# matteocarnelos/microflow-rs

Measured on AMD Instinct MI355X. Metric: inferences/sec (int8) for person_detect.tflite, higher is better.
Workload: dtype i8; 1 GPU; person_detect.tflite batch=65536 per GPU, predict_inner int8->int8, inputs resident in HBM; per_gpu_batch=65536, global_batch=65536, parallelism=batch shard x1, no data-path collective

## Files before the change

microflow_rs_amd/csrc/fused.hip:

```cpp
#include <algorithm>
#include <cmath>
#include <cstdio>
#include <cstring>
#include <memory>

#include "ops_impl.hpp"
#include "wimage.hpp"

namespace mf {

struct FusedImpl {
    enum Kind { DWPW, TAIL, FCSM, STAGE, DWFC, PAIRTAIL, QUAD, CHAIN, FCCHAIN, POOLFC } kind;
    OpImpl *a, *b, *c;
    k::DwPwArgs dwpw;
    k::TailArgs tail;
    std::string name;
    k::StageArgs stage{};
    int stage_pairs = 0;
    std::vector<std::unique_ptr<DevBuf>> stage_w;
    k::DwFcArgs dwfc{};
    k::PairTailArgs pairtail{};
    k::PairFrontArgs pairfront{};
    bool has_front = false;
    k::QuadArgs quad{};
// ... 464 lines not shown
    std::unique_ptr<FusedImpl> f(new FusedImpl{FusedImpl::PAIRTAIL, dw, pairtail->b, pairtail->c, {}, {}, "pair_front_tail<6,6,128,2,256|3,3,256,2>"});
    f->pairtail = t, f->has_front = true, f->epi_mode = magic;
    k::PairFrontArgs &a = f->pairfront;
    a.dw_wmm = df.wmm, a.dwA = df.A, a.dwS = df.S, a.dwK = magic ? kc_with_magic(*f, dw->h_Kc) : df.Kc;
    a.dw_lo = df.lo_f, a.dw_hi = df.hi_f, a.izp4 = df.izp4;
    a.pw_w = plain_pw_image(*f, pw);
    a.pwA = pw->conv.A, a.pwS = pw->conv.S, a.pwK = magic ? kc_with_magic(*f, pw->h_Kc) : pw->conv.Kc;
    a.pw_lo = pw->conv.lo_f, a.pw_hi = pw->conv.hi_f;
    return f.release();
}

static FusedImpl *quad_group(FusedImpl *p1, FusedImpl *p2, const k::DwPwArgs &a, const k::DwPwArgs &b, const char *name, bool mm) {
    const OpSpec &d1 = p1->a->s, &q1 = p1->b->s, &d2 = p2->a->s, &q2 = p2->b->s;
    FusedImpl *f = new FusedImpl{FusedImpl::QUAD, p1->a, p2->b, nullptr, {}, {}, name};
    f->quad.a = a, f->quad.b = b, f->quad_mm = mm;
    f->epi_mode = std::min(pair_mode(a), pair_mode(b));
    f->quad_ops[0] = p1->a, f->quad_ops[1] = p1->b, f->quad_ops[2] = p2->a, f->quad_ops[3] = p2->b;
    const int shp[10] = {d1.H, d1.W, d1.C, d1.sh, q1.N, d2.H, d2.W, d2.C, d2.sh, q2.N};
    for (int i = 0; i < 10; ++i) f->quad_shape[i] = shp[i];
    return f;
}
FusedImpl *fused_quad_create(FusedImpl *p1, FusedImpl *p2) {
    const bool off = switches().no_quad;
    if (off || !p1 || !p2 || p1->kind != FusedImpl::DWPW || p2->kind != FusedImpl::DWPW) return nullptr;
    const OpSpec &d1 = p1->a->s, &q1 = p1->b->s, &d2 = p2->a->s, &q2 = p2->b->s;
    if (p1->a->device != p2->a->device || d1.u8 != d2.u8) return nullptr;
    if (d2.H != q1.H || d2.W != q1.W || d2.C != q1.N) return nullptr;
    if (k::quad_mm_shape(d1.H, d1.W, d1.C, d1.sh, q1.N, d2.H, d2.W, d2.C, d2.sh, q2.N)) {
        if (switches().no_quad_mm) return nullptr;
        k::DwPwArgs a = p1->dwpw, b = p2->dwpw;
        if (pair_mode(a) != 3 || pair_mode(b) != 3) a = pair_args(p1->a, p1->b, 0), b = pair_args(p2->a, p2->b, 0);
        if (!a.dw.wmm || !a.pw.wprep || !b.dw.wmm || !b.pw.wprep) return nullptr;
        if (!a.dw.magic || !a.pw.magic || !b.dw.magic || !b.pw.magic) return nullptr;
        return quad_group(p1, p2, a, b, "quad_mm<12,12,64,1,64|12,12,64,2,128>", true);
    }
    const char *nm = k::quad_name(d1.H, d1.W, d1.C, d1.sh, q1.N, d2.H, d2.W, d2.C, d2.sh, q2.N);
    if (!nm) return nullptr;
    const bool fma = p1->a->fma_strict() && p1->b->fma_strict() && p2->a->fma_strict() && p2->b->fma_strict();
    const k::DwPwArgs a = pair_args(p1->a, p1->b, fma ? 1 : 0), b = pair_args(p2->a, p2->b, fma ? 1 : 0);
    if (!a.dw.wmm || !a.pw.wrr || !b.dw.wmm || !b.pw.wrr) return nullptr;
    if (!a.dw.magic || !a.pw.magic || !b.dw.magic || !b.pw.magic) return nullptr;
    return quad_group(p1, p2, a, b, nm, false);
}

FusedImpl *fused_quad_stem_create(OpImpl *stem, FusedImpl *quad) {
    const bool off = switches().no_penta;
    if (off || !stem || !quad || quad->kind != FusedImpl::QUAD || quad->quad.stem || stem->fast != OpImpl::DW_STEM) return nullptr;
    const OpSpec &t = stem->s, &d1 = quad->a->s;
    if (stem->device != quad->a->device || t.u8 != d1.u8 || stem->force_generic) return nullptr;
    if (t.OH != d1.H || t.OW != d1.W || t.N != d1.C || t.sh != 2 || t.sw != 2 || t.C != 1) return nullptr;
    const int *q = quad->quad_shape;
    const char *nm = k::quad_stem_name(t.H, t.W, q[0], q[1], q[2], q[3], q[4], q[5], q[6], q[7], q[8], q[9]);
    if (!nm || !stem->stem.magic) return nullptr;
    std::unique_ptr<FusedImpl> f(new FusedImpl{FusedImpl::QUAD, stem, quad->b, nullptr, {}, {}, nm});
    f->quad = quad->quad;
    for (int i = 0; i < 10; ++i) f->quad_shape[i] = q[i];
    OpImpl *const *qo = quad->quad_ops;
    const bool fma = stem->fma_strict() && qo[0]->fma_strict() && qo[1]->fma_strict() && qo[2]->fma_strict() && qo[3]->fma_strict();
    f->quad.a = pair_args(qo[0], qo[1], fma ? 1 : 0), f->quad.b = pair_args(qo[2], qo[3], fma ? 1 : 0);
    k::DwStemArgs sa = stem->stem;
    if (fma) sa.use_fma();
    std::vector<uint32_t> tab(152);
    for (int l = 0; l < 64; ++l) tab[(size_t)2 * l] = sa.wmm[l][0], tab[(size_t)2 * l + 1] = sa.wmm[l][1];
    for (int c = 0; c < 8; ++c) {
        memcpy(&tab[(size_t)128 + c], &sa.A[c], 4);
        memcpy(&tab[(size_t)136 + c], &sa.S[c], 4);
        memcpy(&tab[(size_t)144 + c], &sa.Kc[c], 4);
// ... 358 lines not shown
```

microflow_rs_amd/csrc/k_quad_mm.hip:

```cpp
#include "k_common.hpp"

#ifndef MF_QMM_UB
#define MF_QMM_UB 2
#endif
#ifndef MF_QMM_KO
#define MF_QMM_KO 0
#endif
namespace mf {
namespace k {

namespace {
struct Q64 {
    static constexpr int G = 2, NTHR = 512, NWAVE = 8, NQ = 4, LP = 64, ROWB = 768;
    static constexpr int ROW_A = LP + ROWB + LP + 16, TILE_A = 14 * ROW_A, BUF_A = G * TILE_A;
    static constexpr int OPIX_A = 144, NPIX_A = G * OPIX_A, PLANE_A = NPIX_A * 16 + 16;
    static constexpr int ROW_B = LP + ROWB + LP, TILE_B = 14 * ROW_B, BUF_B = G * TILE_B, TS_B = 0x043;
    static constexpr int OPIX_B = 36, NPIX_B = G * OPIX_B, P16_B = 80, PLANE_B = P16_B * 16 + 16;
    static constexpr int OFF_TA = 0;
    static constexpr int OFF_MA = OFF_TA + BUF_A + 512;
    static constexpr int OFF_TB = OFF_MA + NQ * PLANE_A + 64;
    static constexpr int OFF_MB = OFF_TB + BUF_B + 512;
    static constexpr int OFF_C = OFF_MB + NQ * PLANE_B + 64;
    static constexpr int C_A_DW = 0, C_A_PW = 64 * 12, C_B_DW = 2 * 64 * 12, C_B_PW = 3 * 64 * 12, C_BYTES = 3 * 64 * 12 + 128 * 12;
    static constexpr int OFF_Q = OFF_C + C_BYTES;
    static constexpr int LDS = OFF_Q + 16;
};
static_assert(2 * Q64::LDS <= 160 * 1024, "two workgroups per CU");
static_assert(Q64::OFF_MA % 16 == 0 && Q64::OFF_TB % 16 == 0 && Q64::OFF_MB % 16 == 0, "16-byte aligned regions");
}

template <int MG, uint32_t XR4>
__global__ __launch_bounds__(512, 4) void quad_mm_12x12x64(const int8_t *__restrict__ in, int8_t *__restrict__ out, QuadArgs p, int batch) {
    using Z = Q64;
    constexpr int UB = MF_QMM_UB;
    epi_enter<MG>();
    extern __shared__ __attribute__((aligned(16))) uint8_t lds[];
// ... 181 lines not shown
                                                    : requant_pack4<MG, XR4>(acc[t][0], acc[t][1], acc[t][2], acc[t][3], k.a, k.s, p.b.dw.lo_f, p.b.dw.hi_f);
                if (liveB) *(uint32_t *)(lds + mbB + t * 2 * 6 * 16) = d;
            }
        }
        if (!(MF_QMM_KO & 1)) wg_sync();

        if (!(MF_QMM_KO & 4)) {
            constexpr int NC = 5;
            const Consts k = consts(Z::C_B_PW, 128, chB);
            v4i b[NC], acc[NC];
#pragma unroll
            for (int c = 0; c < NC; ++c) {
                const int pix = c * 16 + col, pc = pix < Z::NPIX_B ? pix : Z::NPIX_B - 1;
                b[c] = *(const v4i *)(lds + Z::OFF_MB + g * Z::PLANE_B + pc * 16);
            }
#pragma unroll
            for (int c = 0; c < NC; ++c) acc[c] = __builtin_amdgcn_mfma_i32_16x16x64_i8(AwB, b[c], v4i{k.k.x, k.k.y, k.k.z, k.k.w}, 0, 0, 0);
#pragma unroll
            for (int c = 0; c < NC; ++c) {
                const int pix = c * 16 + col;
                if constexpr (MG == 3) epi_patch_apply(acc[c], prPB, g);
                const uint32_t d = (MF_QMM_KO & 16) ? (uint32_t)(acc[c][0] ^ acc[c][1] ^ acc[c][2] ^ acc[c][3])
                                                    : requant_pack4<MG, XR4>(acc[c][0], acc[c][1], acc[c][2], acc[c][3], k.a, k.s, p.b.pw.lo_f, p.b.pw.hi_f);
                if (pix < Z::NPIX_B) *(uint32_t *)(lds + out_addr(pix, blk * 4 + g) + 4 * tt) = d;
            }
        }
        prev = step, prev_gv = gvalid;
    }
    wg_sync();
    if (prev >= 0) copy_out(prev, prev_gv);
    dq.finish(tid);
}

template <int MG, uint32_t XR4> static void launch_quad_mm_t(const int8_t *in, int8_t *out, const QuadArgs &a, int batch, hipStream_t s) {
    static LaunchState st;
    const int per_cu = prepared(st, quad_mm_12x12x64<MG, XR4>, Q64::NTHR, Q64::LDS);
    const int nsteps = (batch + Q64::G - 1) / Q64::G;
    const int grid = nsteps < 256 * per_cu ? nsteps : 256 * per_cu;
    QuadArgs b = a;
    b.a.dw.qcfg = dq_config(nsteps, grid, dq_est_us((double)batch * (9216 + 4608), (double)batch * (9216 * 2 + 2304 + 4608)));
    b.a.dw.queue = dq_slot(b.a.dw.queue, b.a.dw.qlaunch);
    hipLaunchKernelGGL((quad_mm_12x12x64<MG, XR4>), dim3(grid), dim3(Q64::NTHR), Q64::LDS, s, in, out, b, batch);
}
bool quad_mm_shape(int H, int W, int C, int S, int N, int H2, int W2, int C2, int S2, int N2) {
    return H == 12 && W == 12 && C == 64 && S == 1 && N == 64 && H2 == 12 && W2 == 12 && C2 == 64 && S2 == 2 && N2 == 128;
}
void launch_quad_mm(const int8_t *in, int8_t *out, const QuadArgs &a, int batch, hipStream_t s) {
    const int mg = std::min(std::min(a.a.dw.magic, a.a.pw.magic), std::min(a.b.dw.magic, a.b.pw.magic));
    const bool u8 = a.a.dw.xr != 0;
    if (mg == 3) launch_quad_mm_t<3, 0u>(in, out, a, batch, s);
    else if (u8) {
        if (mg == 2) launch_quad_mm_t<2, 0x80808080u>(in, out, a, batch, s);
        else launch_quad_mm_t<1, 0x80808080u>(in, out, a, batch, s);
    } else {
        if (mg == 2) launch_quad_mm_t<2, 0u>(in, out, a, batch, s);
        else launch_quad_mm_t<1, 0u>(in, out, a, batch, s);
    }
}

}
}
```

microflow_rs_amd/csrc/kernels.hpp:

```cpp
#pragma once
#include <hip/hip_runtime.h>
#include <stddef.h>
#include <stdint.h>

#include <vector>

namespace mf {
namespace k {

struct ConvArgs {
    int H, W, C;
    int N;
    int KH, KW, sh, sw, OH, OW;
    int pad_same;
    int izp;
    float lo_f, hi_f;
    const int8_t *w;
    const int *wzp;
    const float *A;
    const float *S;
    const int *Kc;
    int xr;
};
struct PoolArgs {
// ... 248 lines not shown
    const ChainPair *pairs;
    int npairs, G;
    int lds_bytes, mid_off, q_off;
    int dbuf, dbuf_stride;
    int stage_after;
    int nfill;
    int fill_off[CHAIN_MAX], fill_bytes[CHAIN_MAX];
    uint32_t fill_izp4[CHAIN_MAX];
    int *queue;
    unsigned long *qlaunch;
    int qcfg;
    int KSC;
    int max_cg;
    int resident;
    int nwave;
    double est_us_per_image;
    int magic, xr;
    double hbm_bytes, requant_bytes;
};
bool chain_plan(const ChainGeom *g, int n, ChainPair *pairs, ChainArgs &a, int lds_budget, int force_G = 0, int force_dbuf = -1);
double chain_unfused_us_per_image(const ChainGeom *g, int n);
void chain_rtab(const ChainPair &c, std::vector<int> &out);
void launch_chain(const int8_t *in, int8_t *out, const ChainArgs &a, int batch, hipStream_t s);

struct QuadArgs {
    DwPwArgs a, b;
    const uint32_t *stem;
    uint32_t stem_izp4;
    float stem_lo, stem_hi;
    int stem_magic;
    float in_scale, in_zp_f, in_sat_lo, in_sat_hi, in_rcp;
    uint32_t in_xr4;
    int in_fast, f32_ok;
};
const char *quad_name(int H, int W, int C, int S, int N, int H2, int W2, int C2, int S2, int N2);
const char *quad_stem_name(int SH, int SW, int H, int W, int C, int S, int N, int H2, int W2, int C2, int S2, int N2);
bool launch_quad(int H, int W, int C, int S, int N, int H2, int W2, int C2, int S2, int N2, const int8_t *in, int8_t *out, const QuadArgs &a,
                 int batch, hipStream_t s);
bool quad_mm_shape(int H, int W, int C, int S, int N, int H2, int W2, int C2, int S2, int N2);
void launch_quad_mm(const int8_t *in, int8_t *out, const QuadArgs &a, int batch, hipStream_t s);
bool launch_quad_f32(int H, int W, int C, int S, int N, int H2, int W2, int C2, int S2, int N2, const float *in, int8_t *out, const QuadArgs &a,
                     int batch, hipStream_t s);

struct TailArgs {
    int H, W, C, N;
    int ntaps;
    int tap_off[64];
    float inv_len;
    float pool_c0, pool_c1;
    int pool_lo, pool_hi;
    const int8_t *w;
    const int *wzp;
    const float *A;
    const float *S;
    const int *Kc;
    float lo_f, hi_f;
    const float *exp_table;
    float sm_oscale, sm_ozp_f;
    int pool_bias;
    float pool_sat_lo, pool_sat_hi, sm_sat_lo, sm_sat_hi;
    int xr;
};

struct DwFcGeom {
    static constexpr int H = 49, W = 40, KH = 10, KW = 8, S = 2, OH = 25, OW = 20;
    static constexpr int IMGS = 16;
// ... 291 lines not shown
```

microflow_rs_amd/csrc/mf_switches.hpp:

```cpp
#pragma once
#include <string>
#include <vector>

namespace mf {

struct ChainPlanSeg {
    int len;
    int G;
    int dbuf;
};
bool chain_plan_parse(const char *text, std::vector<ChainPlanSeg> &out, std::string &err);

struct Switches {
    bool dev = false;
    bool no_rt = false;
    bool no_stem_rt = false;
    bool no_chain = false;
    bool chain_no_sp = false;
    bool no_stage = false;
    bool no_fc_rt = false;
    bool no_fc_sparse = false;
    bool no_fc_chain = false;
    bool no_pool_fc = false;
    bool no_conv_gemm = false;
    bool no_dw_gemm = false;
    bool no_dwfc = false;
    bool no_pairtail = false;
    bool no_pair_front = false;
    bool no_quad_mm = false;
    bool no_quad = false;
    bool no_penta = false;
    bool no_f32_group = false;
    int quads = 7;
    bool no_magic = false;
    bool no_sat_pack = false;
    bool no_table = false;
    bool chain_all = false;
    bool chain_force = false;
    bool chain_no_res = false;
    bool conv_mm_256 = false;
    bool no_fma_epi = false;
    bool no_fast_quant_div = false;
    bool dwpw_mm_only = false;
    bool stem_valu = false;
    bool dw_c1_lds = false;
    int dw_alt = -1;
    int dwmm_alt = -1;
    int dwrr_alt = -1;
    int fc_tile = 0;
    bool fc_rowsum_fold = false;
    bool fc_rowsum_prepass = false;
    long long pw_grid = 0;
    int pw_rt_ncap = 64;
    int dw_rt_threads = 0;
    int chain_autotune = -1;
    bool chain_tune_g = true;
    double chain_opcost = 1.0;
    bool chain_dq_auto = false;
    bool chain_plan_set = false;
    std::vector<ChainPlanSeg> chain_plan;
    std::string chain_plan_error;
    bool dq_tune = false;
// ... 15 lines not shown
```

microflow_rs_amd/csrc/ops.hip:

```cpp
#include <algorithm>
#include <array>
#include <cmath>
#include <cstdio>
#include <cstdlib>
#include <cstring>
#include <map>
#include <memory>
#include <mutex>

#include "ops_impl.hpp"
#include "wimage.hpp"

namespace mf {

int dev_count() {
    int n = 0;
    if (hipGetDeviceCount(&n) != hipSuccess) {
        (void)hipGetLastError();
        return 0;
    }
    return n;
}

void dev_require(int device) {
// ... 277 lines not shown
    k::DwC1Args &f = op.dwc1;
    f.H = s.H, f.W = s.W, f.N = s.N, f.KH = s.KH, f.KW = s.KW, f.sh = s.sh, f.sw = s.sw;
    f.OH = s.OH, f.OW = s.OW, f.pad_same = s.pad == MF_PAD_SAME, f.izp = s.izp;
    f.A = op.conv.A, f.S = op.conv.S, f.Kc = op.conv.Kc;
    epi_fields(f, op, c);
    f.KG = (s.KW + 3) / 4;
    f.TWP = ((((s.OW - 1) * s.sw + 3) & ~3) + 4 * (f.KG + 1) + 3) & ~3;
    if (k::dw_c1_supported(f)) {
        op.h_wpack = wimage::build_dw_c1_pack(s.weights, s.KH, s.KW, s.N, f.KG);
        op.d_wprep.upload(op.h_wpack.data(), op.h_wpack.size() * 4);
        f.wpack = op.d_wprep.as<uint32_t>();
        op.fast = OpImpl::DW_C1;
        op.fast_name = "dw_c1_lds";
    }
    return true;
}

bool route_pw_mfma(OpImpl &op, const ConvCtx &c) {
    const OpSpec &s = c.s;
    if (!(!switches().no_table && !c.dw && c.zero_wzp && s.KH == 1 && s.KW == 1 && s.sh == 1 && s.sw == 1 &&
          s.OH == s.H && s.OW == s.W && k::pw_name(s.C, s.N) &&
          (s.C != 8 || ((s.H * s.W) % 2 == 0))))
        return false;
    op.fast = OpImpl::PW_MFMA;
    op.fast_name = k::pw_name(s.C, s.N);
    const std::vector<int8_t> prep = wimage::build_pw_weights(s.weights, s.C, s.N);
    op.d_wprep.upload(prep.data(), prep.size());
    k::PwArgs &f = op.pw;
    f.wprep = op.d_wprep.p, f.A = op.conv.A, f.S = op.conv.S, f.Kc = op.conv.Kc;
    epi_fields(f, op, c);
    f.wrr = nullptr;
    if ((s.C == 8 || s.C == 16 || s.C == 32) && (s.C == 8 ? 2 * s.N : s.N) % 16 == 0) {
        const std::vector<int8_t> rr = wimage::build_pw_rr_weights(s.weights, s.C, s.N);
        op.d_wrr.upload(rr.data(), rr.size());
        f.wrr = op.d_wrr.p;
    }
    return true;
}

bool rt_candidate(const OpImpl &op, const ConvCtx &c) {
    const bool no_rt = switches().no_rt;
    return op.fast == OpImpl::NONE && !no_rt && c.finite;
}

bool route_dw_rt(OpImpl &op, const ConvCtx &c) {
    const OpSpec &s = c.s;
    if (!(rt_candidate(op, c) && c.dw && c.same3x3 && s.C == s.N && k::dw_rt_plan(op.dwrt, s.H, s.W, s.C, s.sh, s.OH, s.OW))) return false;
    op.fast = OpImpl::DW_RT;
    op.rt_wz = c.wz;
    op.fast_name = std::string("dw3x3_rt<") + std::to_string(s.sh) + (op.rt_wz ? ",wzp>" : ">");
    k::DwFastArgs &f = op.dwrt.dw;
    f.w = op.conv.w, f.A = op.conv.A, f.S = op.conv.S, f.Kc = op.conv.Kc, f.wmm = nullptr;
    epi_fields_izp(f, op, c);
    step_queue(f, op);
    op.dwrt.wzp = op.conv.wzp;
    if (!op.rt_wz && (s.C % 16 == 0 || s.C == 8)) {
        const std::vector<int8_t> prep = wimage::build_dw_mm_weights(s.weights, s.C);
        op.d_wprep.upload(prep.data(), prep.size());
        f.wmm = op.d_wprep.p;
    }
    return true;
}

bool route_pw_rt(OpImpl &op, const ConvCtx &c) {
    const OpSpec &s = c.s;
    if (!(rt_candidate(op, c) && !c.dw && s.KH == 1 && s.KW == 1 && s.sh == 1 && s.sw == 1 && s.OH == s.H && s.OW == s.W)) return false;
// ... 658 lines not shown
```

microflow_rs_amd/csrc/switches.cpp:

```cpp
#include "mf_switches.hpp"
#include <cstdlib>
#include <string>

namespace mf {

static bool env_set(const char *name) { return getenv(name) != nullptr; }
static bool env_is(const char *name, char first) { const char *e = getenv(name); return e && e[0] == first; }
static long long env_ll(const char *name, long long dflt) { const char *e = getenv(name); return e ? strtoll(e, nullptr, 0) : dflt; }

bool chain_plan_parse(const char *text, std::vector<ChainPlanSeg> &out, std::string &err) {
    out.clear(), err.clear();
    auto bad = [&](const std::string &why) {
        out.clear();
        err = why;
        return false;
    };
    if (!text || !*text) return bad("empty plan");
    const char *p = text;
    for (;;) {
        int v[3];
        for (int f = 0; f < 3; ++f) {
            const bool neg = *p == '-';
            const char *d = p + (neg ? 1 : 0);
            if (*d < '0' || *d > '9') return bad("entry " + std::to_string(out.size()) + ": expected len:G:dbuf");
// ... 15 lines not shown
        if (s.len == 0 && (s.G != 0 || s.dbuf != -1)) return bad(at + "an unfused pair (len 0) takes G 0 and dbuf -1");
        if (s.len >= 2 && s.dbuf != -1) return bad(at + "double buffering is a single pair's choice (len 1): a chain takes dbuf -1");
        out.push_back(s);
        if (!*p) return true;
        if (*p != ',') return bad(at + "expected ',' or the end");
        ++p;
    }
}

Switches switches_parse() {
    Switches s;
    s.verbose = env_set("MF_VERBOSE");
    s.chain_verbose = env_set("MF_CHAIN_VERBOSE");
    s.dq_verbose = env_set("MF_DQ_VERBOSE");
    s.debug_epi = env_set("MF_DEBUG_EPI");
    s.dev = env_is("MF_DEV", '1');
    if (!s.dev) return s;
    s.no_rt = env_set("MF_NO_RT");
    s.no_stem_rt = env_set("MF_NO_STEM_RT");
    s.no_chain = env_set("MF_NO_CHAIN");
    s.chain_no_sp = env_set("MF_CHAIN_NO_SP");
    s.no_stage = env_set("MF_NO_STAGE");
    s.no_dwfc = env_set("MF_NO_DWFC");
    s.no_fc_rt = env_set("MF_NO_FC_RT");
    s.no_fc_chain = env_set("MF_NO_FC_CHAIN");
    s.no_pool_fc = env_set("MF_NO_POOL_FC");
    s.no_conv_gemm = env_set("MF_NO_CONV_GEMM");
    s.no_dw_gemm = env_set("MF_NO_DW_GEMM");
    s.no_fc_sparse = env_set("MF_NO_FC_SPARSE");
    s.no_pairtail = env_set("MF_NO_PAIRTAIL");
    s.no_quad = env_set("MF_NO_QUAD");
    s.no_pair_front = env_set("MF_NO_PAIR_FRONT");
    s.no_quad_mm = env_set("MF_NO_QUAD_MM");
    s.no_penta = env_set("MF_NO_PENTA");
    s.no_f32_group = env_set("MF_NO_F32_GROUP");
    s.quads = (int)env_ll("MF_QUADS", 7);
    s.no_magic = env_set("MF_NO_MAGIC");
    s.no_sat_pack = env_set("MF_NO_SAT_PACK");
    s.no_table = env_set("MF_NO_TABLE");
    s.chain_all = env_set("MF_CHAIN_ALL");
    s.chain_force = env_set("MF_CHAIN_FORCE");
    s.chain_no_res = env_set("MF_CHAIN_NO_RES");
    s.conv_mm_256 = env_set("MF_CONV_MM_256");
    s.no_fma_epi = env_set("MF_NO_FMA_EPI");
    s.no_fast_quant_div = env_set("MF_NO_FAST_QUANT_DIV");
    s.dwpw_mm_only = env_is("MF_DWPW_IMPL", 'm');
    s.stem_valu = env_is("MF_STEM_IMPL", 'v');
    s.dw_c1_lds = env_is("MF_DW_C1", 'l');
    s.dw_alt = (int)env_ll("MF_DW_ALT", -1);
    s.dwmm_alt = (int)env_ll("MF_DWMM_ALT", -1);
    s.dwrr_alt = (int)env_ll("MF_DWRR_ALT", -1);
    s.fc_tile = (int)env_ll("MF_FC_TILE", 0);
    s.fc_rowsum_fold = env_set("MF_FC_ROWSUM_FOLD");
    s.fc_rowsum_prepass = env_set("MF_FC_ROWSUM_PREPASS");
    s.pw_grid = env_ll("MF_PW_GRID", 0);
    s.pw_rt_ncap = (int)env_ll("MF_PW_RT_NCAP", 64);
    s.dw_rt_threads = (int)env_ll("MF_DW_RT_THREADS", 0);
    s.chain_autotune = !env_set("MF_CHAIN_AUTOTUNE") ? -1 : (env_is("MF_CHAIN_AUTOTUNE", '0') ? 0 : 1);
    s.chain_tune_g = !env_is("MF_CHAIN_TUNE_G", '0');
    if (const char *e = getenv("MF_CHAIN_OPCOST")) s.chain_opcost = atof(e);
    s.chain_dq_auto = env_set("MF_CHAIN_DQ_AUTO");
    if (const char *e = getenv("MF_CHAIN_PLAN")) s.chain_plan_set = true, chain_plan_parse(e, s.chain_plan, s.chain_plan_error);
    s.dq_tune = env_set("MF_DQ_TUNE");
    s.dq_cfg_set = env_set("MF_DQ_CFG");
    s.dq_cfg = (int)env_ll("MF_DQ_CFG", 0);
    if (const char *l = getenv("MF_DQ_CFGS")) s.dq_cfgs = l;
// ... 11 lines not shown
```

microflow_rs_amd/csrc/wimage.cpp:

```cpp
#include "wimage.hpp"

#include <cstring>

namespace mf {
namespace wimage {

std::vector<int8_t> build_pw_weights(const int8_t *w , int K, int N) {
    const int NB = N < 64 ? N : 64, TB = NB / 16, NSPLIT = N / NB;
    const int KS = K < 64 ? 1 : K / 64, Q = K < 64 ? 64 / K : 1;
    std::vector<int8_t> out((size_t)NSPLIT * Q * TB * KS * 64 * 16, 0);
    for (int blk = 0; blk < NSPLIT; ++blk)
        for (int q = 0; q < Q; ++q)
            for (int tt = 0; tt < TB; ++tt)
                for (int ks = 0; ks < KS; ++ks)
                    for (int lane = 0; lane < 64; ++lane) {
                        const int r = lane & 15, g = lane >> 4;
                        const int gr = r >> 2, j = r & 3;
                        const int ch = blk * NB + gr * (NB / 4) + 4 * tt + j;
                        int8_t *dst = &out[(((((size_t)blk * Q + q) * TB + tt) * KS + ks) * 64 + lane) * 16];
                        for (int i = 0; i < 16; ++i) {
                            int k = -1;
                            if (K >= 64) k = ks * 64 + g * 16 + i;
                            else if (K == 32) k = ((g >> 1) == q) ? (g & 1) * 16 + i : -1;
                            else if (K == 16) k = (g == q) ? i : -1;
// ... 81 lines not shown
            for (int pp = 0; pp < P; ++pp) {
                const int tx = P * (g - 1) + pp - S * p + 1;
                if (g < 3 && tx >= 0 && tx <= 2) dst[pp * C + c] = w[(ty * 3 + tx) * C + c];
            }
        }
    return out;
}

std::vector<int8_t> build_pw_rr_weights(const int8_t *w , int K, int N) {
    const bool pair = K == 8;
    const int NT = (pair ? 2 * N : N) / 16;
    std::vector<int8_t> out((size_t)NT * 64 * 8, 0);
    for (int m = 0; m < NT; ++m)
        for (int lane = 0; lane < 64; ++lane) {
            const int r = lane & 15, g = lane >> 4;
            const int gr = r >> 2, i = r & 3;
            const int n = pair ? 8 * (gr & 1) + 4 * m + i : (N / 4) * gr + 4 * m + i;
            int8_t *dst = &out[((size_t)m * 64 + lane) * 8];
            for (int b = 0; b < 8; ++b) {
                int k = -1;
                if (pair) {
                    if (b < 4 && (g >> 1) == (gr >> 1)) k = 4 * (g & 1) + b;
                } else if (b < 4) {
                    k = 4 * g + b;
                } else if (K == 32) {
                    k = 16 + 4 * g + (b - 4);
                }
                dst[b] = k >= 0 && n < N ? w[(size_t)n * K + k] : (int8_t)0;
            }
        }
    return out;
}

std::vector<int8_t> build_pw_rt_weights(const int8_t *w , int K, int N, int group, bool ones) {
    const int Kg = K * group, Ng = N * group, KS = (Kg + 63) / 64, NT = (Ng + 15) / 16;
    std::vector<int8_t> out(((size_t)NT * KS + (ones ? KS : 0)) * 1024, 0);
    for (int nt = 0; nt < NT; ++nt)
        for (int ks = 0; ks < KS; ++ks)
            for (int lane = 0; lane < 64; ++lane) {
                const int row = 16 * nt + (lane & 15), g = lane >> 4;
                if (row >= Ng) continue;
                const int gi = row / N, n = row % N;
                int8_t *dst = &out[(((size_t)nt * KS + ks) * 64 + lane) * 16];
                for (int i = 0; i < 16; ++i) {
                    const int kk = ks * 64 + g * 16 + i;
                    if (kk < Kg && kk / K == gi) dst[i] = w[(size_t)n * K + kk % K];
                }
            }
    if (ones) fill_ones_tile(&out[(size_t)NT * KS * 1024], Kg, KS);
    return out;
}

std::vector<int8_t> build_pw_rt_reg_weights(const int8_t *w , int K, int N, int group, int TB, int NBLK) {
    const int Kg = K * group, Ng = N * group, KS = (Kg + 63) / 64;
    std::vector<int8_t> out((size_t)NBLK * TB * KS * 1024, 0);
    for (int blk = 0; blk < NBLK; ++blk)
        for (int t = 0; t < TB; ++t)
            for (int ks = 0; ks < KS; ++ks)
                for (int lane = 0; lane < 64; ++lane) {
                    const int r = lane & 15, g = lane >> 4;
                    const int row = 16 * TB * blk + 4 * TB * (r >> 2) + 4 * t + (r & 3);
                    if (row >= Ng) continue;
                    const int gi = row / N, n = row % N;
                    int8_t *dst = &out[((((size_t)blk * TB + t) * KS + ks) * 64 + lane) * 16];
                    for (int i = 0; i < 16; ++i) {
                        const int kk = ks * 64 + g * 16 + i;
// ... 67 lines not shown
```

microflow_rs_amd/csrc/wimage.hpp:

```cpp
#pragma once
#include <cstddef>
#include <cstdint>
#include <vector>

namespace mf {
namespace wimage {

std::vector<int8_t> build_pw_weights(const int8_t *w , int K, int N);
std::vector<int8_t> build_dw_mm_weights(const int8_t *w , int C);
std::vector<int8_t> build_dw_sp_weights(const std::vector<int8_t> &dense , int NQ);
std::vector<int8_t> build_dw_mm_rt_weights(const int8_t *w, int KH, int KW, int C, int KS ,
                                           int P = 1);
std::vector<int8_t> build_dw_mm_weights_sp(const int8_t *w , int C, int S);
std::vector<int8_t> build_pw_rr_weights(const int8_t *w , int K, int N);
std::vector<int8_t> build_pw_rt_weights(const int8_t *w , int K, int N, int group, bool ones);
std::vector<int8_t> build_pw_rt_reg_weights(const int8_t *w , int K, int N, int group, int TB, int NBLK);
std::vector<int8_t> build_pw_plain_weights(const int8_t *w, int K, int N);

void fill_ones_tile(int8_t *dst , int K, int KS);
void build_stem_rows(const int8_t *w , int N, uint32_t wrow[3][8]);
void build_stem_mm(const int8_t *w , int N, uint32_t *wmm , int pitch);
std::vector<uint32_t> build_conv_rows_pack(const int8_t *w, bool depthwise, int KH, int KW, int C, int N, int KG, int NP);
inline std::vector<uint32_t> build_dw_c1_pack(const int8_t *w , int KH, int KW, int N, int KG) { return build_conv_rows_pack(w, true, KH, KW, 1, N, KG, 8); }
std::vector<uint32_t> build_conv_rows_mask(int RWB , int KG);

}
}
```

Baseline: 29.78 million inferences/s.

## Add register-resident 64-channel quad_mm kernel that chains depthwise and pointwise outputs in registers

Adds a new variant of the 12x12x64 quad depthwise/pointwise kernel. It runs 256 threads with two workgroups per CU. The first-stage pointwise weights stay in registers, using a new rr64 weight layout for C=64, so the depthwise requantised output feeds the pointwise MFMA straight from registers instead of passing through LDS planes. The second-stage weights move into LDS, MFMA sections are wrapped in s_setprio, and the single epilogue patch is handled as a compile-time template parameter. The aims are to cut LDS traffic and intermediate staging and to raise occupancy, at the cost of higher register pressure and a more complex waitcnt/barrier schedule.

```diff
diff --git a/microflow_rs_amd/csrc/fused.hip b/microflow_rs_amd/csrc/fused.hip
--- a/microflow_rs_amd/csrc/fused.hip
+++ b/microflow_rs_amd/csrc/fused.hip
@@ -520,7 +520,17 @@
         if (pair_mode(a) != 3 || pair_mode(b) != 3) a = pair_args(p1->a, p1->b, 0), b = pair_args(p2->a, p2->b, 0);
         if (!a.dw.wmm || !a.pw.wprep || !b.dw.wmm || !b.pw.wprep) return nullptr;
         if (!a.dw.magic || !a.pw.magic || !b.dw.magic || !b.pw.magic) return nullptr;
-        return quad_group(p1, p2, a, b, "quad_mm<12,12,64,1,64|12,12,64,2,128>", true);
+        const k::EpiPatch &e1 = p1->b->fma_patch;
+        const bool rr = !switches().quad_mm_lds && pair_mode(a) == 3 && pair_mode(b) == 3 && a.pw.wrr && b.pw.wrr && q1.C == 64 && q2.C == 64 &&
+                        p1->a->fma_patch.n == 0 && p2->a->fma_patch.n == 0 && p2->b->fma_patch.n == 0 && e1.n <= 1;
+        FusedImpl *f = quad_group(p1, p2, a, b, rr ? "quad_mm<12,12,64,1,64|12,12,64,2,128>;rr" : "quad_mm<12,12,64,1,64|12,12,64,2,128>", true);
+        f->quad.rr64 = rr ? 1 : 0, f->quad.rr64_ptile = -1;
+        if (rr && e1.n == 1) {
+            const int ch = e1.ch[0];
+            f->quad.rr64_ptile = (ch & 15) >> 2, f->quad.rr64_preg = ch & 3, f->quad.rr64_pgrp = ch >> 4;
+            f->quad.rr64_pP = e1.P[0], f->quad.rr64_pR = e1.R[0];
+        }
+        return f;
     }
     const char *nm = k::quad_name(d1.H, d1.W, d1.C, d1.sh, q1.N, d2.H, d2.W, d2.C, d2.sh, q2.N);
     if (!nm) return nullptr;
diff --git a/microflow_rs_amd/csrc/k_quad_mm.hip b/microflow_rs_amd/csrc/k_quad_mm.hip
--- a/microflow_rs_amd/csrc/k_quad_mm.hip
+++ b/microflow_rs_amd/csrc/k_quad_mm.hip
@@ -1,7 +1,15 @@
 #include "k_common.hpp"
+
+#include <type_traits>
 
 #ifndef MF_QMM_UB
 #define MF_QMM_UB 2
+#endif
+#ifndef MF_R64_PRIO
+#define MF_R64_PRIO 1
+#endif
+#ifndef MF_R64_KO
+#define MF_R64_KO 0
 #endif
 #ifndef MF_QMM_KO
 #define MF_QMM_KO 0
@@ -249,6 +257,266 @@
     dq.finish(tid);
 }
 
+namespace {
+struct R64 {
+    static constexpr int G = 2, NTHR = 256, NWAVE = 4, LP = 64, ROWB = 768;
+    static constexpr int ROW_A = Q64::ROW_A, TILE_A = Q64::TILE_A, BUF_A = Q64::BUF_A;
+    static constexpr int ROW_B = Q64::ROW_B, TILE_B = Q64::TILE_B, BUF_B = Q64::BUF_B, TS_B = Q64::TS_B;
+    static constexpr int OFF_TA = 0, OFF_TB = BUF_A + 512, OFF_C = OFF_TB + BUF_B + 512;
+    static constexpr int C_A_DW = Q64::C_A_DW, C_A_PW = Q64::C_A_PW, C_B_DW = Q64::C_B_DW, C_B_PW = Q64::C_B_PW, C_BYTES = Q64::C_BYTES;
+    static constexpr int OFF_WD = OFF_C + C_BYTES, OFF_WP = OFF_WD + 12 * 1024;
+    static constexpr int OFF_Q = OFF_WP + 8 * 1024, LDS = OFF_Q + 16;
+};
+static_assert(2 * R64::LDS <= 160 * 1024 && R64::OFF_TB % 16 == 0 && R64::OFF_C % 16 == 0, "two workgroups per CU, 16-byte aligned regions");
+__device__ __forceinline__ void rr64_barrier_raw() {
+    mf_jitter();
+    asm volatile("s_waitcnt lgkmcnt(0)\n\ts_barrier" ::: "memory");
+    mf_jitter();
+}
+}
+
+template <int MG, uint32_t XR4, int PM>
+__global__ __launch_bounds__(256, 2) void quad_mm_12x12x64_rr(const int8_t *__restrict__ in, int8_t *__restrict__ out, QuadArgs p, int batch) {
+    using Z = R64;
+    static_assert(MG == 3 || PM < 0, "patched accumulators exist in the single-fma form only");
+    epi_enter<MG>();
+    extern __shared__ __attribute__((aligned(16))) uint8_t lds[];
+    const int tid = threadIdx.x, lane = tid & 63;
+    const int wave = __builtin_amdgcn_readfirstlane(tid >> 6);
+    DynSteps dq;
+    dq.init(lds + Z::OFF_Q, p.a.dw.queue, tid, p.a.dw.qcfg);
+    for (int i = tid; i < (Z::BUF_A + 512) / 16; i += Z::NTHR)
+        ((uint4 *)(lds + Z::OFF_TA))[i] = make_uint4(p.a.dw.izp4, p.a.dw.izp4, p.a.dw.izp4, p.a.dw.izp4);
+    for (int i = tid; i < (Z::BUF_B + 512) / 16; i += Z::NTHR)
+        ((uint4 *)(lds + Z::OFF_TB))[i] = make_uint4(p.b.dw.izp4, p.b.dw.izp4, p.b.dw.izp4, p.b.dw.izp4);
+    {
+        auto put = [&](int off, int n, const float *A, const float *S, const int *K) {
+            for (int i = tid; i < n; i += Z::NTHR) {
+                ((float *)(lds + Z::OFF_C + off))[i] = A[i], ((float *)(lds + Z::OFF_C + off))[n + i] = S[i];
+                ((int *)(lds + Z::OFF_C + off))[2 * n + i] = K[i] + (MG != 0 ? MF_MAGIC_I : 0);
+            }
+        };
+        put(Z::C_A_DW, 64, p.a.dw.A, p.a.dw.S, p.a.dw.Kc), put(Z::C_A_PW, 64, p.a.pw.A, p.a.pw.S, p.a.pw.Kc);
+        put(Z::C_B_DW, 64, p.b.dw.A, p.b.dw.S, p.b.dw.Kc), put(Z::C_B_PW, 128, p.b.pw.A, p.b.pw.S, p.b.pw.Kc);
+    }
+    struct Consts {
+        float4 a, s;
+        int4 k;
+    };
+    auto consts = [&](int off, int n, int ch) {
+        Consts c;
+        c.a = *(const float4 *)(lds + Z::OFF_C + off + ch * 4), c.s = *(const float4 *)(lds + Z::OFF_C + off + (n + ch) * 4);
+        c.k = *(const int4 *)(lds + Z::OFF_C + off + (2 * n + ch) * 4);
+        return c;
+    };
+    const int col = lane & 15, g = lane >> 4;
+    const int cyA = col & 3, cxA = col >> 2;
+    const int tbA = Z::OFF_TA + cyA * Z::ROW_A + Z::LP + (cxA + g - 1) * 64;
+    const int dbA = Z::OFF_TB + (cyA + 1) * Z::ROW_B + Z::LP + cxA * 64;
+    const int cxB = col & 7, cyB = col >> 3, xlB = cxB * 2 + g - 1;
+    int tbB[4];
+#pragma unroll
+    for (int q = 0; q < 4; ++q) tbB[q] = Z::OFF_TB + cyB * 2 * Z::ROW_B + Z::LP + xlB * 64 + 16 * (q ^ tile_swz<Z::TS_B>(xlB));
+    const int obB = (cyB * 6 + cxB) * 128 + 32 * g;
+    const bool liveB = cxB < 6;
+    const int rw = wave;
+    const bool xA = rw < 2, xB = rw >= 2;
+    int offA[5], dofA[5], swA[5], offB[2], oofB[2], hB[2];
+#pragma unroll
+    for (int t = 0; t < 5; ++t) {
+        const int iu = (t < 4 || xA) ? 4 * t + rw : rw, h = iu / 9, r = iu - 9 * h, uy = r / 3, ux = r - 3 * uy;
+        offA[t] = h * Z::TILE_A + uy * 4 * Z::ROW_A + ux * 256, dofA[t] = h * Z::TILE_B + uy * 4 * Z::ROW_B + ux * 256;
+        swA[t] = 16 * ux;
+    }
+#pragma unroll
+    for (int t = 0; t < 2; ++t) {
+        const int iu = t == 0 ? rw : (xB ? rw + 2 : rw), h = iu / 3, r = iu - 3 * h;
+        offB[t] = h * Z::TILE_B + r * 4 * Z::ROW_B, oofB[t] = (h * 36 + r * 12) * 128, hB[t] = h;
+    }
+    v4i AdA[4][3], AwA[4];
+#pragma unroll
+    for (int q = 0; q < 4; ++q)
+#pragma unroll
+        for (int ty = 0; ty < 3; ++ty) AdA[q][ty] = ((const v4i *)p.a.dw.wmm)[(q * 3 + ty) * 64 + lane];
+#pragma unroll
+    for (int m = 0; m < 4; ++m) AwA[m] = ((const v4i *)p.a.pw.wrr)[m * 64 + lane];
+    for (int i = tid; i < 12 * 64; i += Z::NTHR) ((v4i *)(lds + Z::OFF_WD))[i] = ((const v4i *)p.b.dw.wmm)[i];
+    for (int i = tid; i < 8 * 64; i += Z::NTHR) ((v4i *)(lds + Z::OFF_WP))[i] = ((const v4i *)p.b.pw.wrr)[i];
+    v4i pcmp = {0, 0, 0, 0};
+    if constexpr (PM >= 0) {
+        const int P = g == p.rr64_pgrp ? p.rr64_pP : 0;
+        pcmp = v4i{p.rr64_preg == 0 ? P : 0, p.rr64_preg == 1 ? P : 0, p.rr64_preg == 2 ? P : 0, p.rr64_preg == 3 ? P : 0};
+    }
+    const int prepl = p.rr64_pR;
+    wg_sync();
+
+    auto stage = [&](int st) {
+#pragma unroll
+        for (int k = 0; k < 6; ++k) {
+            const int r = k * Z::NWAVE + wave, gi = r / 12, y = r % 12;
+            if (st * Z::G + gi < batch && lane < 48)
+                dma16(in + ((size_t)(st * Z::G + gi) * 9216 + y * Z::ROWB + lane * 16), lds + Z::OFF_TA + gi * Z::TILE_A + (y + 1) * Z::ROW_A + Z::LP);
+        }
+    };
+    auto phase_a = [&](auto nu_c) {
+        constexpr int NU = decltype(nu_c)::value;
+        uint32_t d[NU][4], pk[NU][4];
+        v4i b[NU][3], bn[NU][3];
+        auto taps = [&](v4i (&t)[NU][3], int q) {
+#pragma unroll
+            for (int u = 0; u < NU; ++u)
+#pragma unroll
+                for (int ty = 0; ty < 3; ++ty) t[u][ty] = *(const v4i *)(lds + tbA + 16 * q + offA[u] + ty * Z::ROW_A);
+        };
+        taps(b, 0);
+        Consts k = consts(Z::C_A_DW, 64, 4 * g), kn = k;
+#pragma unroll
+        for (int q = 0; q < 4; ++q) {
+            v4i acc[NU];
+#pragma unroll
+            for (int u = 0; u < NU; ++u) acc[u] = v4i{k.k.x, k.k.y, k.k.z, k.k.w};
+#if MF_R64_PRIO
+            __builtin_amdgcn_s_setprio(MF_R64_PRIO);
+#endif
+#pragma unroll
+            for (int ty = 0; ty < 3; ++ty)
+#pragma unroll
+                for (int u = 0; u < NU; ++u) acc[u] = __builtin_amdgcn_mfma_i32_16x16x64_i8(AdA[q][ty], b[u][ty], acc[u], 0, 0, 0);
+#if MF_R64_PRIO
+            __builtin_amdgcn_s_setprio(0);
+#endif
+            if (q < 3) taps(bn, q + 1), kn = consts(Z::C_A_DW, 64, 16 * (q + 1) + 4 * g);
+            else kn = consts(Z::C_A_PW, 64, 16 * g);
+#pragma unroll
+            for (int u = 0; u < NU; ++u) d[u][q] = requant_pack4<MG, XR4>(acc[u][0], acc[u][1], acc[u][2], acc[u][3], k.a, k.s, p.a.dw.lo_f, p.a.dw.hi_f);
+#pragma unroll
+            for (int u = 0; u < NU; ++u)
+#pragma unroll
+                for (int ty = 0; ty < 3; ++ty) b[u][ty] = bn[u][ty];
+            k = kn;
+        }
+#pragma unroll
+        for (int m = 0; m < 4; ++m) {
+            v4i acc[NU];
+#pragma unroll
+            for (int u = 0; u < NU; ++u)
+                acc[u] = __builtin_amdgcn_mfma_i32_16x16x64_i8(AwA[m], v4i{(int)d[u][0], (int)d[u][1], (int)d[u][2], (int)d[u][3]}, v4i{k.k.x, k.k.y, k.k.z, k.k.w}, 0, 0, 0);
+            if (m < 3) kn = consts(Z::C_A_PW, 64, 16 * g + 4 * (m + 1));
+#pragma unroll
+            for (int u = 0; u < NU; ++u) {
+                if (PM == m && !MF_EPI_PATCH_KO) {
+#pragma unroll
+                    for (int j = 0; j < 4; ++j) acc[u][j] = acc[u][j] == pcmp[j] ? prepl : acc[u][j];
+                }
+                pk[u][m] = requant_pack4<MG, XR4>(acc[u][0], acc[u][1], acc[u][2], acc[u][3], k.a, k.s, p.a.pw.lo_f, p.a.pw.hi_f);
+            }
+            k = kn;
+        }
+#pragma unroll
+        for (int u = 0; u < NU; ++u) *(uint4 *)(lds + dbA + dofA[u] + ((16 * g) ^ swA[u])) = make_uint4(pk[u][0], pk[u][1], pk[u][2], pk[u][3]);
+    };
+    auto phase_b = [&](auto nu_c, int8_t *ob, int gvalid) {
+        constexpr int NU = decltype(nu_c)::value;
+        uint32_t d[NU][4], pk[NU][8];
+        v4i b[NU][3], bn[NU][3], Ad[3], Adn[3];
+        auto taps = [&](v4i (&t)[NU][3], v4i (&A)[3], int q) {
+#pragma unroll
+            for (int ty = 0; ty < 3; ++ty) A[ty] = ((const v4i *)(lds + Z::OFF_WD))[(q * 3 + ty) * 64 + lane];
+#pragma unroll
+            for (int u = 0; u < NU; ++u)
+#pragma unroll
+                for (int ty = 0; ty < 3; ++ty) t[u][ty] = *(const v4i *)(lds + tbB[q] + offB[u] + ty * Z::ROW_B);
+        };
+        taps(b, Ad, 0);
+        Consts k = consts(Z::C_B_DW, 64, 4 * g), kn = k;
+        v4i Aw = {0, 0, 0, 0}, Awn = Aw;
+#pragma unroll
+        for (int q = 0; q < 4; ++q) {
+            v4i acc[NU];
+#pragma unroll
+            for (int u = 0; u < NU; ++u) acc[u] = v4i{k.k.x, k.k.y, k.k.z, k.k.w};
+#if MF_R64_PRIO
+            __builtin_amdgcn_s_setprio(MF_R64_PRIO);
+#endif
+#pragma unroll
+            for (int ty = 0; ty < 3; ++ty)
+#pragma unroll
+                for (int u = 0; u < NU; ++u) acc[u] = __builtin_amdgcn_mfma_i32_16x16x64_i8(Ad[ty], b[u][ty], acc[u], 0, 0, 0);
+#if MF_R64_PRIO
+            __builtin_amdgcn_s_setprio(0);
+#endif
+            if (q < 3) taps(bn, Adn, q + 1), kn = consts(Z::C_B_DW, 64, 16 * (q + 1) + 4 * g);
+            else kn = consts(Z::C_B_PW, 128, 32 * g), Aw = ((const v4i *)(lds + Z::OFF_WP))[lane];
+#pragma unroll
+            for (int u = 0; u < NU; ++u) d[u][q] = requant_pack4<MG, XR4>(acc[u][0], acc[u][1], acc[u][2], acc[u][3], k.a, k.s, p.b.dw.lo_f, p.b.dw.hi_f);
+#pragma unroll
+            for (int ty = 0; ty < 3; ++ty) {
+                Ad[ty] = Adn[ty];
+#pragma unroll
+                for (int u = 0; u < NU; ++u) b[u][ty] = bn[u][ty];
+            }
+            k = kn;
+        }
+#pragma unroll
+        for (int m = 0; m < 8; ++m) {
+            v4i acc[NU];
+#pragma unroll
+            for (int u = 0; u < NU; ++u)
+                acc[u] = __builtin_amdgcn_mfma_i32_16x16x64_i8(Aw, v4i{(int)d[u][0], (int)d[u][1], (int)d[u][2], (int)d[u][3]}, v4i{k.k.x, k.k.y, k.k.z, k.k.w}, 0, 0, 0);
+            if (m < 7) kn = consts(Z::C_B_PW, 128, 32 * g + 4 * (m + 1)), Awn = ((const v4i *)(lds + Z::OFF_WP))[(m + 1) * 64 + lane];
+#pragma unroll
+            for (int u = 0; u < NU; ++u) pk[u][m] = requant_pack4<MG, XR4>(acc[u][0], acc[u][1], acc[u][2], acc[u][3], k.a, k.s, p.b.pw.lo_f, p.b.pw.hi_f);
+            k = kn, Aw = Awn;
+        }
+#pragma unroll
+        for (int u = 0; u < NU; ++u)
+            if (liveB && hB[u] < gvalid) {
+                st_out(ob + oofB[u], make_uint4(pk[u][0], pk[u][1], pk[u][2], pk[u][3]));
+                st_out(ob + oofB[u] + 16, make_uint4(pk[u][4], pk[u][5], pk[u][6], pk[u][7]));
+            }
+    };
+
+    const int nsteps = (batch + Z::G - 1) / Z::G;
+    if (dq.step < nsteps) stage(dq.step);
+    bool counted = false;
+    int ko_steps = 0;
+    for (; dq.step < nsteps; dq.advance(tid)) {
+        const int step = dq.step;
+        if (counted && !(MF_R64_KO & 4)) {
+            if (xB) asm volatile("s_waitcnt vmcnt(4)" ::: "memory");
+            else asm volatile("s_waitcnt vmcnt(2)" ::: "memory");
+        } else {
+            asm volatile("s_waitcnt vmcnt(0)" ::: "memory");
+        }
+        rr64_barrier_raw();
+        dq.top(tid);
+        const int gvalid = min(Z::G, batch - step * Z::G);
+        if (xA) phase_a(std::integral_constant<int, 5>{});
+        else phase_a(std::integral_constant<int, 4>{});
+        if (!(MF_R64_KO & 1)) wg_sync();
+        if (dq.nxt < nsteps && !((MF_R64_KO & 2) && ko_steps > 0)) stage(dq.nxt);
+        int8_t *ob = out + (size_t)step * Z::G * 36 * 128 + obB;
+        if (!(MF_R64_KO & 4)) {
+            if (xB) phase_b(std::integral_constant<int, 2>{}, ob, gvalid);
+            else phase_b(std::integral_constant<int, 1>{}, ob, gvalid);
+        }
+        counted = gvalid == Z::G;
+        ++ko_steps;
+    }
+    dq.finish(tid);
+}
+
+template <int PM> static void launch_quad_mm_rr_t(const int8_t *in, int8_t *out, const QuadArgs &a, int batch, hipStream_t s) {
+    static LaunchState st;
+    const int per_cu = prepared(st, quad_mm_12x12x64_rr<3, 0u, PM>, R64::NTHR, R64::LDS);
+    const int nsteps = (batch + R64::G - 1) / R64::G;
+    const int grid = nsteps < 256 * per_cu ? nsteps : 256 * per_cu;
+    QuadArgs b = a;
+    b.a.dw.qcfg = dq_config(nsteps, grid, dq_est_us((double)batch * (9216 + 4608), (double)batch * (9216 * 2 + 2304 + 4608)));
+    b.a.dw.queue = dq_slot(b.a.dw.queue, b.a.dw.qlaunch);
+    hipLaunchKernelGGL((quad_mm_12x12x64_rr<3, 0u, PM>), dim3(grid), dim3(R64::NTHR), R64::LDS, s, in, out, b, batch);
+}
+
 template <int MG, uint32_t XR4> static void launch_quad_mm_t(const int8_t *in, int8_t *out, const QuadArgs &a, int batch, hipStream_t s) {
     static LaunchState st;
     const int per_cu = prepared(st, quad_mm_12x12x64<MG, XR4>, Q64::NTHR, Q64::LDS);
@@ -265,6 +533,15 @@
 void launch_quad_mm(const int8_t *in, int8_t *out, const QuadArgs &a, int batch, hipStream_t s) {
     const int mg = std::min(std::min(a.a.dw.magic, a.a.pw.magic), std::min(a.b.dw.magic, a.b.pw.magic));
     const bool u8 = a.a.dw.xr != 0;
+    if (a.rr64 && mg == 3) {
+        switch (a.rr64_ptile) {
+        case 0: return launch_quad_mm_rr_t<0>(in, out, a, batch, s);
+        case 1: return launch_quad_mm_rr_t<1>(in, out, a, batch, s);
+        case 2: return launch_quad_mm_rr_t<2>(in, out, a, batch, s);
+        case 3: return launch_quad_mm_rr_t<3>(in, out, a, batch, s);
+        default: return launch_quad_mm_rr_t<-1>(in, out, a, batch, s);
+        }
+    }
     if (mg == 3) launch_quad_mm_t<3, 0u>(in, out, a, batch, s);
     else if (u8) {
         if (mg == 2) launch_quad_mm_t<2, 0x80808080u>(in, out, a, batch, s);
diff --git a/microflow_rs_amd/csrc/kernels.hpp b/microflow_rs_amd/csrc/kernels.hpp
--- a/microflow_rs_amd/csrc/kernels.hpp
+++ b/microflow_rs_amd/csrc/kernels.hpp
@@ -304,6 +304,7 @@
     float in_scale, in_zp_f, in_sat_lo, in_sat_hi, in_rcp;
     uint32_t in_xr4;
     int in_fast, f32_ok;
+    int rr64, rr64_ptile, rr64_preg, rr64_pgrp, rr64_pP, rr64_pR;
 };
 const char *quad_name(int H, int W, int C, int S, int N, int H2, int W2, int C2, int S2, int N2);
 const char *quad_stem_name(int SH, int SW, int H, int W, int C, int S, int N, int H2, int W2, int C2, int S2, int N2);
diff --git a/microflow_rs_amd/csrc/mf_switches.hpp b/microflow_rs_amd/csrc/mf_switches.hpp
--- a/microflow_rs_amd/csrc/mf_switches.hpp
+++ b/microflow_rs_amd/csrc/mf_switches.hpp
@@ -28,6 +28,7 @@
     bool no_pairtail = false;
     bool no_pair_front = false;
     bool no_quad_mm = false;
+    bool quad_mm_lds = false;
     bool no_quad = false;
     bool no_penta = false;
     bool no_f32_group = false;
diff --git a/microflow_rs_amd/csrc/ops.hip b/microflow_rs_amd/csrc/ops.hip
--- a/microflow_rs_amd/csrc/ops.hip
+++ b/microflow_rs_amd/csrc/ops.hip
@@ -333,6 +333,10 @@
     f.wrr = nullptr;
     if ((s.C == 8 || s.C == 16 || s.C == 32) && (s.C == 8 ? 2 * s.N : s.N) % 16 == 0) {
         const std::vector<int8_t> rr = wimage::build_pw_rr_weights(s.weights, s.C, s.N);
+        op.d_wrr.upload(rr.data(), rr.size());
+        f.wrr = op.d_wrr.p;
+    } else if (s.C == 64 && s.N % 16 == 0) {
+        const std::vector<int8_t> rr = wimage::build_pw_rr64_weights(s.weights, s.N);
         op.d_wrr.upload(rr.data(), rr.size());
         f.wrr = op.d_wrr.p;
     }
diff --git a/microflow_rs_amd/csrc/switches.cpp b/microflow_rs_amd/csrc/switches.cpp
--- a/microflow_rs_amd/csrc/switches.cpp
+++ b/microflow_rs_amd/csrc/switches.cpp
@@ -71,6 +71,7 @@
     s.no_quad = env_set("MF_NO_QUAD");
     s.no_pair_front = env_set("MF_NO_PAIR_FRONT");
     s.no_quad_mm = env_set("MF_NO_QUAD_MM");
+    s.quad_mm_lds = env_set("MF_QUAD_MM_LDS");
     s.no_penta = env_set("MF_NO_PENTA");
     s.no_f32_group = env_set("MF_NO_F32_GROUP");
     s.quads = (int)env_ll("MF_QUADS", 7);
diff --git a/microflow_rs_amd/csrc/wimage.cpp b/microflow_rs_amd/csrc/wimage.cpp
--- a/microflow_rs_amd/csrc/wimage.cpp
+++ b/microflow_rs_amd/csrc/wimage.cpp
@@ -137,6 +137,20 @@
     return out;
 }
 
+std::vector<int8_t> build_pw_rr64_weights(const int8_t *w , int N) {
+    const int NT = N / 16;
+    std::vector<int8_t> out((size_t)NT * 64 * 16, 0);
+    for (int m = 0; m < NT; ++m)
+        for (int lane = 0; lane < 64; ++lane) {
+            const int r = lane & 15, g = lane >> 4;
+            const int n = (N / 4) * (r >> 2) + 4 * m + (r & 3);
+            int8_t *dst = &out[((size_t)m * 64 + lane) * 16];
+            for (int q = 0; q < 4; ++q)
+                for (int j = 0; j < 4; ++j) dst[4 * q + j] = w[(size_t)n * 64 + 16 * q + 4 * g + j];
+        }
+    return out;
+}
+
 std::vector<int8_t> build_pw_rt_weights(const int8_t *w , int K, int N, int group, bool ones) {
     const int Kg = K * group, Ng = N * group, KS = (Kg + 63) / 64, NT = (Ng + 15) / 16;
     std::vector<int8_t> out(((size_t)NT * KS + (ones ? KS : 0)) * 1024, 0);
diff --git a/microflow_rs_amd/csrc/wimage.hpp b/microflow_rs_amd/csrc/wimage.hpp
--- a/microflow_rs_amd/csrc/wimage.hpp
+++ b/microflow_rs_amd/csrc/wimage.hpp
@@ -13,6 +13,7 @@
                                            int P = 1);
 std::vector<int8_t> build_dw_mm_weights_sp(const int8_t *w , int C, int S);
 std::vector<int8_t> build_pw_rr_weights(const int8_t *w , int K, int N);
+std::vector<int8_t> build_pw_rr64_weights(const int8_t *w , int N);
 std::vector<int8_t> build_pw_rt_weights(const int8_t *w , int K, int N, int group, bool ones);
 std::vector<int8_t> build_pw_rt_reg_weights(const int8_t *w , int K, int N, int group, int TB, int NBLK);
 std::vector<int8_t> build_pw_plain_weights(const int8_t *w, int K, int N);
```

New measurement: 29.99 million inferences/s, median of 6. No clear change (+0.7%).
